# RIKEN-RCCS/GEMMul8

Measured on AMD Instinct MI355X. Metric: emulated DGEMM TFLOPS (N=8192, moduli=14), higher is better.
Workload: dtype int8

## Files before the change

### gemmul8_amd/csrc/oz2_driver.hip

```cpp
#include <hip/hip_runtime.h>
#include <stdint.h>
#include <stdio.h>
#include <stdlib.h>
#include <string.h>

#include <algorithm>

#include <atomic>
#include <mutex>

#include "../../include/gemmul8_c.h"
#include "oz2_gemm_common.hpp"
#include "oz2_kernels.h"
#include "oz2_knobs.hpp"

using namespace oz2;

namespace {

inline char* align256(void* p) {
    uintptr_t x = reinterpret_cast<uintptr_t>(p);
    x = (x + 255) & ~uintptr_t(255);
    return reinterpret_cast<char*>(x);
}
inline int norm_op(int op) {
    if (op >= 111 && op <= 113) return op - 111;
    return op;
}
inline size_t low_size(int) { return 1; }
inline size_t mid_size(int backend, bool cplx) { return (backend == kINT8 ? 1 : 2) * (cplx ? 2 : 1); }

static inline bool moduli_ok(int dtype, unsigned N) { return N >= 2 && N <= (is_f32(dtype) ? 13u : 20u); }

static inline bool f8_concat_ok(size_t k, size_t m, size_t n, size_t kp) { return k <= 32768 && 2 * (m + n) * kp <= ((size_t)384 << 20); }

#define OZ2_HIP(expr)                       \
    do {                                    \
        hipError_t e__ = (expr);            \
        if (e__ != hipSuccess) return (int)e__; \
    } while (0)

struct Timer {
    hipEvent_t ev[4];
    bool made = false, ok = false;
};
Timer* thread_timer() {
    constexpr int kMaxDev = 64;
    static thread_local Timer t[kMaxDev];
    int dev = 0;
    if (hipGetDevice(&dev) != hipSuccess || dev < 0 || dev >= kMaxDev) return nullptr;
    Timer& T = t[dev];
    if (!T.made) {
        T.made = T.ok = true;
        for (auto& e : T.ev)
            if (hipEventCreate(&e) != hipSuccess) T.ok = false;
    }
    return T.ok ? &T : nullptr;
}

}

static bool scalars_on_device(const void* alpha);

namespace oz2 {
static Knobs parse_knobs() {
    Knobs k;
    auto num = [](const char* name, int dflt) {
        const char* s = getenv(name);
        return s && *s ? atoi(s) : dflt;
    };
    if (const char* e = getenv("GEMMUL8_EPI_NT"); e && (e[0] == '0' || e[0] == '1') && !e[1]) k.epi_nt = e[0] - '0';
    if (const int t = num("GEMMUL8_BOUND_TILE", 0); t == 128 || t == 256) k.bound_tile = t;
    if (num("GEMMUL8_CPLX_BOUND_LAUNCHES", 1) == 2) k.cplx_bound_launches = 2;
    if (const int c = num("GEMMUL8_CPLX_CHUNK", 0); c >= 1) k.cplx_chunk = c;
    if (const char* e = getenv("GEMMUL8_CRT_KERNEL")) k.crt_kernel = e[0] == 'd' ? 1 : e[0] == 'r' ? 2 : 0;
    if (const int c = num("GEMMUL8_GEMM_CUS", 0); c >= 8) k.gemm_cus = c & ~7;
    if (const char* e = getenv("GEMMUL8_FP8_FUSED"); e && e[0] == '0') k.fp8_fused = 0;
    if (const char* e = getenv("GEMMUL8_FP8_PLANES")) k.fp8_planes = e[0] == 'e' ? 1 : 0;
    if (const char* e = getenv("GEMMUL8_SCALE_FOLD"); e && e[0] == '0') k.scale_fold = 0;
    if (const char* e = getenv("GEMMUL8_BOUNDS_ONE_READ"); e && (e[0] == '0' || e[0] == '1') && !e[1]) k.bounds_one_read = e[0] - '0';
    if (const char* e = getenv("GEMMUL8_CRT_PANELS"); e && atoi(e) > 1) {
        k.crt_panels = std::min(atoi(e), 256);
        k.crt_panels_ring = e[strlen(e) - 1] == 'r';
    }
    if (const char* e = getenv("GEMMUL8_MAP_COLBLOCK"); e && *e) k.map_colblock = atoi(e) > 0 ? atoi(e) : 0;
    return k;
}
static std::atomic<const Knobs*> g_knobs{nullptr};
static std::mutex g_knobs_mtx;
void reload_knobs() {
    std::lock_guard<std::mutex> lk(g_knobs_mtx);
    g_knobs.store(new Knobs(parse_knobs()), std::memory_order_release);
}
const Knobs& knobs() {
    const Knobs* k = g_knobs.load(std::memory_order_acquire);
    if (!k) {
        std::lock_guard<std::mutex> lk(g_knobs_mtx);
        k = g_knobs.load(std::memory_order_acquire);
        if (!k) g_knobs.store(k = new Knobs(parse_knobs()), std::memory_order_release);
    }
    return *k;
}
}

extern "C" {

void gemmul8_reload_knobs(void) { oz2::reload_knobs(); }

static std::atomic<int> g_nonfinite_mode{0};
int gemmul8_set_nonfinite_mode(int mode) {
    if (mode < 0 || mode > 1) return GEMMUL8_E_ARG;
    return g_nonfinite_mode.exchange(mode);
}

int gemmul8_set_fp8_bound_mode(int mode) {
    if (mode < 0 || mode > 2) return GEMMUL8_E_ARG;
    const int old = get_f8_bound_mode();
    set_f8_bound_mode(mode);
    return old;
}

int gemmul8_abi_version(void) { return GEMMUL8_ABI_VERSION; }
size_t gemmul8_layout_bytes(void) { return sizeof(gemmul8_layout); }

const char* gemmul8_version(void) { return "gemmul8-mi355x 0.5 (gfx950; v_mfma_i32_16x16x64_i8 / v_mfma_scale_f32_16x16x128_f8f6f4, fused epilogues)"; }

size_t gemmul8_work_size(int is_complex, int backend, size_t m, size_t n, size_t k, unsigned N, int enA, int enB, size_t* wA,
                         size_t* wB) {
    const size_t kp = padding256(k), mp = padding256(m);
    const size_t sizeA = kp * mp, sizeB = kp * n, sizeC = mp * n;
    const size_t nm = num_mat(backend, N);
    const size_t parts = is_complex ? 3 : 1;
    const size_t midsz = mid_size(backend, is_complex != 0);
    const size_t nhi = (backend == kINT8 ? 1 : 3) * parts;
    const size_t lwork = size_t(1) << 25;
    size_t tA = 255, tB = 255, tC = 255;
    tA += sizeA * (nm + (enA ? 1 : 0)) * parts + 2 * mp;
    tB += sizeB * (nm + (enB ? 1 : 0)) * parts + 2 * padding256(n);
    tC += midsz * sizeC * (N - 1) + std::max(lwork, midsz * sizeC);
    tC += 4 * sizeC * nhi;
    if (wA) *wA = tA;
    if (wB) *wB = tB;
    return tA + tB + tC;
}

int gemmul8_get_layout(int dtype, int backend, size_t m, size_t n, size_t k, unsigned N, void* work, void* workA, void* workB,
                       int enA, int enB, gemmul8_layout* L) {
    if (!L || !work) return GEMMUL8_E_ARG;
    if (!moduli_ok(dtype, N)) return GEMMUL8_E_NUM_MODULI;
    const bool cplx = is_complex(dtype);
    memset(L, 0, sizeof(*L));
    L->kp = padding256(k);
    L->mp = padding256(m);
    L->num_mat = num_mat(backend, N);
    L->parts = cplx ? 3 : 1;
    L->sizeA = L->kp * L->mp;
    L->sizeB = L->kp * n;
    L->sizeC = L->mp * n;
    const size_t offsetA = L->sizeA * L->num_mat, offsetB = L->sizeB * L->num_mat;
    const size_t size_vecA = L->mp, size_vecB = padding256(n);
    char* w = align256(work);
    char* wa = workA ? align256(workA) : nullptr;
    char* wb = workB ? align256(workB) : nullptr;
    char* A_lo = wa ? wa : w;
    char* sftA = A_lo + L->parts * offsetA + (enA ? L->parts * L->sizeA : 0);
    char* B_lo = wb ? wb : (wa ? w : sftA + 2 * size_vecA);
    char* sftB = B_lo + L->parts * offsetB + (enB ? L->parts * L->sizeB : 0);
    char* C_mid = wb ? (wa ? w : sftA + 2 * size_vecA) : sftB + 2 * size_vecB;
    const size_t midsz = mid_size(backend, cplx);
    char* work_native = C_mid + (N - 1) * L->sizeC * midsz;
    const size_t native_sz = std::max(size_t(1) << 25, midsz * L->sizeC);
    char* C_hi = work_native + native_sz;
    const size_t hi_bytes = 4 * L->sizeC * (backend == kINT8 ? 1 : 3) * L->parts;
    L->A_lo = A_lo;
    L->B_lo = B_lo;
    L->part_strideA = offsetA;
    L->part_strideB = offsetB;
    L->A_bound = enA ? A_lo + L->parts * offsetA : A_lo;
    L->B_bound = enB ? B_lo + L->parts * offsetB : B_lo;
    L->sftA = reinterpret_cast<int16_t*>(sftA);
    L->sftB = reinterpret_cast<int16_t*>(sftB);
    L->C_mid = C_mid;
    const size_t tail = (native_sz - midsz * L->sizeC) & ~size_t(255);
    L->scratch = C_hi - tail;
    L->scratch_bytes = tail + hi_bytes;
    L->lo_format = (backend == kFP8 && !enA && !enB && f6_planes_ok(n)) ? 1 : 0;
    return GEMMUL8_OK;
}

static inline size_t scale_fixed_bytes(size_t mp, size_t np) { return (4 * (mp + np) + 2 * (mp + np) + 255) / 256 * 256; }
static inline size_t scale_scratch_bytes(size_t mp, size_t np) { return scale_fixed_bytes(mp, np) + 8 * (mp + np); }
static int scale_scratch(const gemmul8_layout* L, size_t n, int** rowmax, int** colmax, void** amax, int16_t** s0A = nullptr, int16_t** s0B = nullptr) {
    const size_t np = padding256(n);
    if (L->scratch_bytes < scale_scratch_bytes(L->mp, np)) return GEMMUL8_E_ARG;
    *rowmax = (int*)L->scratch;
    *colmax = *rowmax + L->mp;
    int16_t* s0 = (int16_t*)(*colmax + np);
    if (s0A) *s0A = s0;
    if (s0B) *s0B = s0 + L->mp;
    *amax = (char*)L->scratch + scale_fixed_bytes(L->mp, np);
    return GEMMUL8_OK;
}

static int bound_gemm_i8(hipStream_t stream, bool cplx, const gemmul8_layout* L, size_t m, size_t ncols, const int8_t* Ab, const int8_t* Bb, int* rowmax, int* colmax) {
    if (!cplx) {
        const int8_t* As[1] = {Ab};
        const int8_t* Bs[1] = {Bb};
        OZ2_HIP(launch_gemm_i8_max(stream, 1, As, Bs, L->kp, m, ncols, rowmax, colmax));
    } else {
        const int8_t* As[3] = {Ab, Ab + L->sizeA, Ab + 2 * L->sizeA};
        const int8_t* Bs[3] = {Bb + L->sizeB, Bb, Bb + 2 * L->sizeB};
        const bool two_launches = knobs().cplx_bound_launches == 2;
        if (two_launches) {
            OZ2_HIP(launch_gemm_i8_max(stream, 2, As, Bs, L->kp, m, ncols, rowmax, colmax));
            OZ2_HIP(launch_gemm_i8_max(stream, 3, As, Bs, L->kp, m, ncols, rowmax, colmax));
        } else {
            OZ2_HIP(launch_gemm_i8_max(stream, 3, As, Bs, L->kp, m, ncols, rowmax, colmax, 2));
        }
    }
    return GEMMUL8_OK;
}

struct SymSide {
    bool onB;
    int form;
    bool herm;
    bool conj = false;
};
constexpr size_t kOneReadMinRows = 8192;
static int scale_bounds_nf(void* stream_, int dtype, int backend, int op_A, int op_B, size_t m, size_t n, size_t k, const void* A, size_t lda,
                           const void* B, size_t ldb, unsigned N, size_t col_begin, size_t col_end, const gemmul8_layout* L, int skipA, int skipB,
                           bool nf, const SymSide* sym = nullptr) {
    hipStream_t stream = (hipStream_t)stream_;
// ... 893 lines not shown
```

### gemmul8_amd/csrc/oz2_knobs.hpp

```cpp
#pragma once

namespace oz2 {

struct Knobs {
    int epi_nt = -1;
    int bound_tile = 0;
    int cplx_bound_launches = 1;
    int cplx_chunk = 0;
    int crt_kernel = 0;
    int fp8_planes = 0;
    int fp8_fused = 1;
    int gemm_cus = 0;
    int crt_panels = 0;
    int crt_panels_ring = 0;
    int scale_fold = 1;
    int bounds_one_read = -1;
    int map_colblock = -1;
};
const Knobs& knobs();
void reload_knobs();

}
```

### gemmul8_amd/csrc/oz2_scale.hip

```cpp
#include <hip/hip_runtime.h>
#include <limits.h>
#include <stdint.h>

#include <algorithm>
#include <type_traits>

#include "oz2_kernels.h"

namespace oz2 {

ModTable make_mod_table(int backend) {
    ModTable T;
    for (int t = 0; t < 20; ++t) {
        const int p = backend == kINT8 ? GEMMUL8_MODULI_INT8[t] : GEMMUL8_MODULI_FP8[t];
        T.mc[t].p = p;
        T.mc[t].invp = 1.0f / (float)p;
        unsigned c[16];
        long long pw = 1;
        for (int i = 0; i < 16; ++i) {
            c[i] = i < 15 ? (unsigned)(pw % p) : 0u;
            pw = (pw % p) * 256;
        }
        for (int i = 0; i < 4; ++i) {
            unsigned lo = 0, hi = 0;
// ... 780 lines not shown
                    for (int e = 0; e < RPL; ++e) {
                        const T q = (lrow + e < a.rows) ? x[kg * a.ld + e] : (T)0;
                        __builtin_memcpy((char*)&v + e * sizeof(T), &q, sizeof(T));
                    }
                }
            }
            b[it] = v;
        }
    };
    auto to_lds = [&](const V4 (&b)[NL]) {
#pragma unroll
        for (int it = 0; it < NL; ++it) {
            const int kk = ky + KY * it;
#pragma unroll
            for (int e = 0; e < RPL; ++e) __builtin_memcpy(&tile[RPL * rp + e][kk], (const char*)&b[it] + e * sizeof(T), sizeof(T));
        }
    };
    auto consume = [&]<bool FAST>(unsigned t) {
#pragma unroll
        for (int p = 0; p < NP; ++p) {
            const int rl = p * RPP + rg;
            T v[4];
            T lm = 0;
#pragma unroll
            for (int e = 0; e < 4; ++e) {
                v[e] = tile[rl][c * 4 + e];
                const T ax = sizeof(T) == 8 ? (T)fabs((double)v[e]) : (T)fabsf((float)v[e]);
                lm = ax > lm ? ax : lm;
                if constexpr (sizeof(T) == 8) {
                    const unsigned hw = (unsigned)__double2hiint((double)ax);
                    mnk[p] = (v[e] != (T)0 && hw < mnk[p]) ? hw : mnk[p];
                }
            }
            int key = lm == (T)0 ? kNone : lm == (T)INFINITY ? INT_MAX : ilogb0(lm);
#pragma unroll
            for (int off = CH / 2; off > 0; off >>= 1) key = max(key, __shfl_xor(key, off));
            const int prev = ex[p];
            ex[p] = max(prev, key);
            if (c == 0) step[rl][t] = (unsigned char)(prev == kNone ? 0 : min(min(ex[p], 4096) - min(prev, 4096), 255));
            if (FAST || r0 + rl < a.rows) emit4<T, MODE_BOUND>(a, r0 + rl, (size_t)t * TK + c * 4, v, ex[p] == kNone ? 5 : 5 - min(ex[p], 4096));
        }
    };
    unsigned tdone = 0;
    if (r0 + TR <= a.rows && ((reinterpret_cast<uintptr_t>(X + r0) | (a.ld * sizeof(T))) & 15u) == 0) {
        auto fetch = [&](unsigned t, V4 (&b)[NL]) {
#pragma unroll
            for (int it = 0; it < NL; ++it) b[it] = __builtin_nontemporal_load((const V4*)(x + ((size_t)t * TK + ky + KY * it) * a.ld));
        };
        V4 buf[D][NL];
#pragma unroll
        for (int j = 0; j < D; ++j) {
#pragma unroll
            for (int it = 0; it < NL; ++it) buf[j][it] = V4{0u, 0u, 0u, 0u};
            if ((unsigned)j < nfull) fetch((unsigned)j, buf[j]);
        }
        for (unsigned t0 = 0; t0 < nfull; t0 += D) {
#pragma unroll
            for (int j = 0; j < D; ++j) {
                const unsigned t = t0 + j;
                if (t < nfull) {
                    to_lds(buf[j]);
                    if (t + D < nfull) fetch(t + D, buf[j]);
                    __syncthreads();
                    consume.template operator()<true>(t);
                    __syncthreads();
                }
            }
        }
        tdone = nfull;
    }
    for (unsigned t = tdone; t < nkt; ++t) {
        V4 b[NL];
        fetch_guarded(t, b);
        to_lds(b);
        __syncthreads();
        consume.template operator()<false>(t);
        __syncthreads();
    }
#pragma unroll
    for (int p = 0; p < NP; ++p) {
        const int rl = p * RPP + rg;
        const size_t row = r0 + rl;
        if (row >= a.rows) continue;
        const int s0 = ex[p] == kNone ? 5 : ex[p] == INT_MAX ? 5 - ilogb0((T)INFINITY) : 5 - ex[p];
        if (c == 0) {
            ((int16_t*)((char*)a.sft0 + OZ2_ZW))[row] = (int16_t)s0;
            if (a.sft0_keep) ((int16_t*)((char*)a.sft0_keep + OZ2_ZW))[row] = (int16_t)s0;
        }
        bool hazard = ex[p] == INT_MAX;
        if constexpr (sizeof(T) == 8) {
            unsigned mk = mnk[p];
#pragma unroll
            for (int off = CH / 2; off > 0; off >>= 1) mk = min(mk, (unsigned)__shfl_xor((int)mk, off));
            const int emin = (mk >> 20) == 0 ? -1074 : (int)(mk >> 20) - 1023;
            hazard = hazard || (ex[p] != kNone && mk != 0xFFFFFFFFu && s0 + emin < -1022);
        }
        if (hazard) {
            for (unsigned t = 0; t < nkt; ++t) {
                const size_t k0 = (size_t)t * TK + c * 4;
                T v[4];
#pragma unroll
                for (int e = 0; e < 4; ++e) v[e] = (k0 + e < a.k) ? X[(k0 + e) * a.ld + row] : (T)0;
                emit4<T, MODE_BOUND>(a, row, k0, v, s0);
            }
            continue;
        }
        unsigned d = 0;
        for (int t = (int)nkt - 1; t >= 1; --t) {
            d = min(d + step[rl][t], 64u);
            if (d == 0) continue;
            unsigned* q = (unsigned*)(a.lo + OZ2_ZW + row * a.kp + (size_t)(t - 1) * TK + c * 4);
            const unsigned w = *q;
            *q = d >= 8 ? (((w + 0x7F7F7F7Fu) >> 7) & 0x01010101u) : (((w + ((1u << d) - 1u) * 0x01010101u) >> d) & ((0xFFu >> d) * 0x01010101u));
        }
    }
}

template <typename T> __global__ void __launch_bounds__(256) extract_pair_kernel(const StageArgs a, const StageArgs b, const unsigned nA, const int kmA, const int kmB) {
    if (a.zero_words) {
        unsigned* zp = (unsigned*)((char*)a.zero_p + OZ2_ZW);
        for (unsigned i = blockIdx.x * 256u + threadIdx.x; i < a.zero_words; i += gridDim.x * 256u) zp[i] = 0u;
    }
    if (blockIdx.x < nA) {
        if (kmA) stage_kmajor_body<T, MODE_BOUND>(a, blockIdx.x);
        else stage_strided_body<T, MODE_BOUND>(a, blockIdx.x);
    } else {
        if (kmB) stage_kmajor_body<T, MODE_BOUND>(b, blockIdx.x - nA);
        else stage_strided_body<T, MODE_BOUND>(b, blockIdx.x - nA);
    }
}
enum { FORM_STRIDED = 0, FORM_KMAJOR = 1, FORM_PANEL = 2 };
template <typename T> __device__ __forceinline__ void extract_body(const StageArgs& a, const unsigned bid, const int form) {
    if (form == FORM_KMAJOR) return stage_kmajor_body<T, MODE_BOUND>(a, bid);
    if (form == FORM_PANEL) return stage_panel_body<T>(a, bid);
    stage_strided_body<T, MODE_BOUND>(a, bid);
}
template <typename T> __global__ void __launch_bounds__(256) extract_panel_pair_kernel(const StageArgs a, const StageArgs b, const unsigned nA, const int fA, const int fB) {
    if (a.zero_words) {
        unsigned* zp = (unsigned*)((char*)a.zero_p + OZ2_ZW);
        for (unsigned i = blockIdx.x * 256u + threadIdx.x; i < a.zero_words; i += gridDim.x * 256u) zp[i] = 0u;
    }
    if (blockIdx.x < nA) extract_body<T>(a, blockIdx.x, fA);
    else extract_body<T>(b, blockIdx.x - nA, fB);
}
template <typename T> __global__ void __launch_bounds__(256) quantise_pair_kernel(const StageArgs a, const StageArgs b, const unsigned nA, const int kmA, const int kmB) {
    if (blockIdx.x < nA) {
        if (kmA) stage_kmajor_body<T, MODE_MOD>(a, blockIdx.x);
        else stage_strided_body<T, MODE_MOD>(a, blockIdx.x);
    } else {
        if (kmB) stage_kmajor_body<T, MODE_MOD>(b, blockIdx.x - nA);
        else stage_strided_body<T, MODE_MOD>(b, blockIdx.x - nA);
    }
}
template <typename T> __global__ void __launch_bounds__(256) quantise_twin_kernel(const StageArgs a, const int km) {
    static_assert(ET<T>::cplx, "complex operands");
    if (km) stage_kmajor_body<T, MODE_MOD, true>(a, blockIdx.x);
    else stage_strided_body<T, MODE_MOD, true>(a, blockIdx.x);
}
template <typename T> __global__ void __launch_bounds__(256) extract_seg2_kernel(const StageArgs a, const int km) {
    if (a.zero_words) {
        unsigned* zp = (unsigned*)((char*)a.zero_p + OZ2_ZW);
        for (unsigned i = blockIdx.x * 256u + threadIdx.x; i < a.zero_words; i += gridDim.x * 256u) zp[i] = 0u;
    }
    if (km) stage_kmajor_seg2_body<T, MODE_BOUND>(a, blockIdx.x);
    else stage_strided_body<T, MODE_BOUND, false, true>(a, blockIdx.x);
}
template <typename T> __global__ void __launch_bounds__(256) quantise_seg2_kernel(const StageArgs a, const int km) {
    if (km) stage_kmajor_seg2_body<T, MODE_MOD>(a, blockIdx.x);
    else stage_strided_body<T, MODE_MOD, false, true>(a, blockIdx.x);
}
static_assert(2 * sizeof(StageArgs) + 16 <= 4096, "two argument blocks must fit the 4 KiB kernel-argument segment");

typedef float v16f __attribute__((ext_vector_type(16)));
typedef unsigned v6u __attribute__((ext_vector_type(6)));
template <typename T> __device__ __forceinline__ void stage_f6_body(const StageArgs& a, const unsigned bid, const bool kmajor, char* tile ) {
    static_assert(!ET<T>::cplx, "real operands");
    constexpr int EPL = 16 / (int)sizeof(T);
    constexpr int CH = 128 / (int)sizeof(T);
    const unsigned lane = threadIdx.x & 63u, q = threadIdx.x >> 6;
    const unsigned nks = (unsigned)(a.kp / 128), nrb = (unsigned)((a.rows + 63) / 64);
    unsigned rb, kt;
    if (kmajor) rb = bid / nks, kt = bid - rb * nks;
    else kt = bid / nrb, rb = bid - kt * nrb;
    const size_t r0 = (size_t)rb * 64, row = r0 + lane, k0 = (size_t)kt * 128 + (size_t)q * 32;
    const T* X = (const T*)((const char*)a.X + OZ2_ZX);
    typedef unsigned V4 __attribute__((ext_vector_type(4)));
    T v[32];
    if (kmajor) {
        const unsigned pc = lane & 7u, pr = lane >> 3;
#pragma unroll
        for (int c = 0; c < 32 / CH; ++c) {
            V4 buf[8];
#pragma unroll
            for (int j = 0; j < 8; ++j) {
                const size_t r = r0 + pr + 8 * j, kk = k0 + (size_t)c * CH + (size_t)pc * EPL;
                const T* src = X + r * a.ld + kk;
                V4 t = {0u, 0u, 0u, 0u};
                if (r < a.rows) {
                    if (kk + EPL <= a.k && (reinterpret_cast<uintptr_t>(src) & 15u) == 0) {
                        t = __builtin_nontemporal_load((const V4*)src);
                    } else {
                        T e[EPL];
#pragma unroll
                        for (int u = 0; u < EPL; ++u) e[u] = kk + u < a.k ? src[u] : ET<T>::zero();
                        __builtin_memcpy(&t, e, 16);
                    }
                }
                buf[j] = t;
            }
            if (c > 0) __builtin_amdgcn_wave_barrier();
#pragma unroll
            for (int j = 0; j < 8; ++j) *(V4*)(tile + (pr + 8 * j) * 144 + pc * 16) = buf[j];
            __builtin_amdgcn_wave_barrier();
#pragma unroll
            for (int i = 0; i < 8; ++i) {
                const V4 t = *(const V4*)(tile + lane * 144 + i * 16);
                __builtin_memcpy(&v[c * CH + i * EPL], &t, 16);
            }
        }
    } else {
        const T* src = X + row;
#pragma unroll
        for (int kk = 0; kk < 32; ++kk) {
            const size_t kg = k0 + kk;
            v[kk] = (row < a.rows && kg < a.k) ? __builtin_nontemporal_load(src + kg * a.ld) : ET<T>::zero();
        }
    }
    if (row >= a.rows) return;
    int s = OZ2_ROW_SHIFT(a, row, k0 == 0);
    if (a.nf && s == kNonfiniteShift) {
#pragma unroll
        for (int e = 0; e < 32; ++e) v[e] = ET<T>::zero();
        s = 0;
    }
    using XS = typename std::conditional<sizeof(T) == 4, float, double>::type;
    XS xs[32];
    bool big = false;
#pragma unroll
    for (int e = 0; e < 32; ++e) {
        if constexpr (sizeof(T) == 4) xs[e] = truncf(ldexpf(v[e], s));
        else xs[e] = trunc(ldexp((double)v[e], s));
        big |= fabs((double)xs[e]) >= 0x1.0p53;
    }
    const unsigned tb = (unsigned)(row >> 8), r = (unsigned)row & 255u;
    const unsigned rp = tb == a.f6_last ? a.f6_rp_last : 256u;
    int8_t* const panel = a.lo + OZ2_ZW + (size_t)tb * 256u * (a.kp / 4 * 3) + (size_t)kt * rp * 96u;
    int8_t* const ox = panel + (size_t)(q * rp + r) * 16u;
    int8_t* const oy = panel + 64u * (size_t)rp + (size_t)((q >> 1) * 2u * rp + 2u * r + (q & 1u)) * 8u;
    auto put = [&](int plane, const float (&w)[32]) {
        v16f ev, od;
#pragma unroll
        for (int i = 0; i < 16; ++i) ev[i] = w[2 * i], od[i] = w[2 * i + 1];
        const v6u c = __builtin_amdgcn_cvt_scalef32_2xpk16_fp6_f32(ev, od, 8.0f);
        typedef unsigned V2 __attribute__((ext_vector_type(2)));
        *(V4*)(ox + (size_t)plane * a.plane_stride) = V4{c[0], c[1], c[2], c[3]};
        *(V2*)(oy + (size_t)plane * a.plane_stride) = V2{c[4], c[5]};
    };
    auto run = [&]<bool BIG>() {
        for (int t = a.t_begin; t < a.t_end; t += 2) {
            const double P = a.pairP[(t - a.t_begin) >> 1], invP = a.pairInvP[(t - a.t_begin) >> 1];
            float Rf[32];
#pragma unroll
            for (int g8 = 0; g8 < 4; ++g8) {
#pragma unroll
                for (int e = 8 * g8; e < 8 * g8 + 8; ++e) {
                    const double x = (double)xs[e];
                    double R = fma(-rint(x * invP), P, x);
                    if constexpr (BIG) R = fma(-rint(R * invP), P, R);
                    Rf[e] = (float)R;
                }
                __builtin_amdgcn_sched_barrier(0);
            }
#pragma unroll 1
            for (int u = 0; u < 2; ++u) {
                const int tt = t + u;
                if (tt >= a.t_end) break;
                const ModConst mc = a.mt.mc[tt];
                const float pf = (float)mc.p;
                const bool even = !(mc.p & 1);
                const bool sqm = tt < 6;
                float lo[32], hi[32];
                if (even) {
                    asm volatile("" ::: "memory");
#pragma unroll
                    for (int e = 0; e < 32; ++e) {
                        const float qq = fmaf(Rf[e], mc.invp, 12582912.0f) - 12582912.0f;
                        const float rr = fmaf(-qq, pf, Rf[e]);
                        lo[e] = rr == -0.5f * pf ? 0.5f * pf : rr;
                    }
                } else {
#pragma unroll
                    for (int g8 = 0; g8 < 4; ++g8) {
#pragma unroll
                        for (int e = 8 * g8; e < 8 * g8 + 8; ++e) {
                            const float qq = fmaf(Rf[e], mc.invp, 12582912.0f) - 12582912.0f;
                            lo[e] = fmaf(-qq, pf, Rf[e]);
                        }
                        __builtin_amdgcn_sched_barrier(0);
                    }
                }
                if (sqm) {
                    const float sq = (float)a.sqrtp[tt], inv = 1.0f / sq;
#pragma unroll
                    for (int g8 = 0; g8 < 4; ++g8) {
#pragma unroll
                        for (int e = 8 * g8; e < 8 * g8 + 8; ++e) {
// ... 187 lines not shown
    };
    const AmaxOperand a = mk(A), b = mk(B);
    const size_t nA = (size_t)a.row_groups * a.parts, nB = (size_t)b.row_groups * b.parts;
    if (nA + nB == 0) return hipSuccess;
    if (nA + nB > 0x7FFFFFFFull) return hipErrorInvalidConfiguration;
    hipLaunchKernelGGL(amax_pair_kernel<T>, dim3((unsigned)(nA + nB), 1, g_batch.batch), dim3(256), 0, stream, a, b, (unsigned)nA, k, g_batch.ws);
    return hipGetLastError();
}
static hipError_t launch_amax_sym_pair(hipStream_t stream, int dtype, size_t k, const ExtractOperand& A, const ExtractOperand& B);
static hipError_t launch_extract_sym_pair(hipStream_t stream, int dtype, int backend, size_t k, size_t kp, const ExtractOperand& A, const ExtractOperand& B,
                                          void* zero_p, size_t zero_bytes);
static hipError_t launch_fast_shift_sym_pair(hipStream_t stream, int dtype, int backend, unsigned N, size_t k, const QuantOperand& A, const QuantOperand& B);
static hipError_t launch_quantise_sym_pair(hipStream_t stream, int dtype, int backend, int t_begin, int t_end, size_t k, size_t kp, const QuantOperand& A,
                                           const QuantOperand& B);

hipError_t launch_amax_pair(hipStream_t stream, int dtype, size_t k, const ExtractOperand& A, const ExtractOperand& B) {
    if (A.sym || B.sym) return launch_amax_sym_pair(stream, dtype, k, A, B);
    switch (dtype) {
    case kF32: return launch_amax_pair_t<float>(stream, k, A, B);
    case kF64: return launch_amax_pair_t<double>(stream, k, A, B);
    case kC32: return launch_amax_pair_t<float2>(stream, k, A, B);
    case kC64: return launch_amax_pair_t<double2>(stream, k, A, B);
    }
    return hipErrorInvalidValue;
}
template <typename T> static size_t extract_blocks(int form, const StageArgs& a) {
    if (form == FORM_PANEL) return (a.rows + StageTile<T>::TR - 1) / StageTile<T>::TR;
    return stage_blocks<T, MODE_BOUND>(form == FORM_KMAJOR, a);
}
template <typename T> static hipError_t launch_extract_pair_t(hipStream_t stream, int kmA, StageArgs a, int kmB, const StageArgs& b, void* zero_p, size_t zero_bytes) {
    const size_t nA = extract_blocks<T>(kmA, a), nB = extract_blocks<T>(kmB, b);
    if (nA + nB == 0) return zero_bytes ? launch_zero(stream, zero_p, zero_bytes) : hipSuccess;
    if (nA + nB > 0x7FFFFFFFull) return hipErrorInvalidConfiguration;
    if (zero_p && zero_bytes) a.zero_p = (unsigned*)zero_p, a.zero_words = (unsigned)(zero_bytes / 4);
    if constexpr (!ET<T>::cplx) {
        if (kmA == FORM_PANEL || kmB == FORM_PANEL) {
            hipLaunchKernelGGL(extract_panel_pair_kernel<T>, dim3((unsigned)(nA + nB), 1, g_batch.batch), dim3(256), 0, stream, a, b, (unsigned)nA, kmA, kmB);
            return hipGetLastError();
        }
    }
    hipLaunchKernelGGL(extract_pair_kernel<T>, dim3((unsigned)(nA + nB), 1, g_batch.batch), dim3(256), 0, stream, a, b, (unsigned)nA, kmA, kmB);
    return hipGetLastError();
}
bool extract_one_read_ok(int dtype, int backend, size_t kp) {
    return (dtype == kF32 || dtype == kF64) && backend == kINT8 && g_batch.batch == 1 && kp / StageTile<double>::TK <= (size_t)kPanelMaxTiles;
}
hipError_t launch_extract_pair(hipStream_t stream, int dtype, int backend, size_t k, size_t kp, const ExtractOperand& A, const ExtractOperand& B, void* zero_p,
                               size_t zero_bytes) {
    if (A.sym || B.sym) return launch_extract_sym_pair(stream, dtype, backend, k, kp, A, B, zero_p, zero_bytes);
    const StageArgs a = extract_args(backend, k, kp, A), b = extract_args(backend, k, kp, B);
    auto form = [&](const ExtractOperand& o) { return o.kmajor ? FORM_KMAJOR : o.one_read ? FORM_PANEL : FORM_STRIDED; };
    if ((A.one_read || B.one_read) && !extract_one_read_ok(dtype, backend, kp)) return hipErrorInvalidValue;
    const int fA = form(A), fB = form(B);
    switch (dtype) {
    case kF32: return launch_extract_pair_t<float>(stream, fA, a, fB, b, zero_p, zero_bytes);
    case kF64: return launch_extract_pair_t<double>(stream, fA, a, fB, b, zero_p, zero_bytes);
    case kC32: return launch_extract_pair_t<float2>(stream, fA, a, fB, b, zero_p, zero_bytes);
    case kC64: return launch_extract_pair_t<double2>(stream, fA, a, fB, b, zero_p, zero_bytes);
    }
    return hipErrorInvalidValue;
}

static StageArgs quantise_args(int backend, int t_begin, int t_end, size_t k, size_t kp, const QuantOperand& o) {
    StageArgs a{};
    a.bx = o.xstride;
    a.bw = g_batch.ws;
    a.X = o.X;
    a.ld = o.ld;
    a.rows = o.rows;
    a.k = k;
    a.kp = kp;
    a.lo = o.lo;
    a.plane_stride = o.plane_stride;
    a.part_stride = o.part_stride;
    a.sft = o.sft;
    if (o.fin_max) {
        a.fin_sft0 = o.fin_sft0;
        a.fin_max = o.fin_max;
        a.fin_out = o.sft;
        a.fin_log2P = o.fin_log2P;
        a.fin_float_max = backend == kFP8 ? 1 : 0;
    }
    a.backend = backend;
    a.conj = o.conj;
    a.nf = o.nf ? 1 : 0;
    a.t_begin = t_begin;
    a.t_end = t_end;
    a.mt = make_mod_table(backend);
    for (int t = t_begin, j = 0; t < t_end && j < 10; t += 2, ++j) {
        const double P = (double)a.mt.mc[t].p * (t + 1 < t_end ? (double)a.mt.mc[t + 1].p : 1.0);
        a.pairP[j] = P;
        a.pairInvP[j] = 1.0 / P;
    }
    for (int t = 0; t < 6; ++t) a.sqrtp[t] = GEMMUL8_SQRT_MODULI_FP8[t];
    if (backend == kFP8 && o.f6_rows > 0) {
        a.f6 = 1;
        a.f6_last = (unsigned)((o.f6_rows - 1) / 256);
        a.f6_rp_last = (unsigned)((o.f6_rows - 256 * (size_t)a.f6_last + 15) / 16 * 16);
    }
    return a;
}

static hipError_t launch_quantise_twin(hipStream_t stream, int dtype, int t_begin, int t_end, size_t k, size_t kp, const QuantOperand& A) {
    StageArgs a = quantise_args(kINT8, t_begin, t_end, k, kp, A);
    a.lo2 = A.lo2, a.plane_stride2 = A.plane_stride2, a.part_stride2 = A.part_stride2;
    const size_t nA = dtype == kC32 ? stage_blocks<float2, MODE_MOD>(A.kmajor, a) : stage_blocks<double2, MODE_MOD>(A.kmajor, a);
    if (nA > 0x7FFFFFFFull) return hipErrorInvalidConfiguration;
    const dim3 grid((unsigned)nA, 1, g_batch.batch);
    if (dtype == kC32) hipLaunchKernelGGL(quantise_twin_kernel<float2>, grid, dim3(256), 0, stream, a, (int)A.kmajor);
    else hipLaunchKernelGGL(quantise_twin_kernel<double2>, grid, dim3(256), 0, stream, a, (int)A.kmajor);
    return hipGetLastError();
}

template <typename T, int MODE> static size_t seg2_blocks(bool kmajor, const StageArgs& a) {
    if (kmajor) return a.rows * ((MODE == MODE_MOD && sizeof(T) <= 8) ? 2 * ((a.kp + 1023) / 1024) : 1);
    return 2 * (a.kp / StageTile<T>::TK) * ((a.rows + StageTile<T>::TR - 1) / StageTile<T>::TR);
}
static void seg2_args(StageArgs& a, size_t kp, const Seg2Planes& S) {
    a.X2 = S.X2, a.ld2 = S.ld2, a.pitch = 2 * kp;
    a.lo2 = S.lo2, a.plane_stride2 = S.plane_stride2, a.part_stride2 = S.part_stride2;
}
template <typename T, int MODE> static hipError_t launch_seg2_t(hipStream_t stream, bool kmajor, const StageArgs& a) {
    const size_t nb = seg2_blocks<T, MODE>(kmajor, a);
    if (nb == 0 || nb > 0x7FFFFFFFull) return hipErrorInvalidConfiguration;
    if constexpr (MODE == MODE_BOUND) hipLaunchKernelGGL(extract_seg2_kernel<T>, dim3((unsigned)nb), dim3(256), 0, stream, a, (int)kmajor);
    else hipLaunchKernelGGL(quantise_seg2_kernel<T>, dim3((unsigned)nb), dim3(256), 0, stream, a, (int)kmajor);
    return hipGetLastError();
}
template <int MODE> static hipError_t launch_seg2(hipStream_t stream, int dtype, bool kmajor, const StageArgs& a) {
    if (g_batch.batch != 1 || a.rows == 0 || a.kp % 256 != 0 || !a.X2 || !a.lo2) return hipErrorInvalidValue;
    switch (dtype) {
    case kF32: return launch_seg2_t<float, MODE>(stream, kmajor, a);
    case kF64: return launch_seg2_t<double, MODE>(stream, kmajor, a);
    case kC32: return launch_seg2_t<float2, MODE>(stream, kmajor, a);
    case kC64: return launch_seg2_t<double2, MODE>(stream, kmajor, a);
    }
    return hipErrorInvalidValue;
}
hipError_t launch_extract_seg2(hipStream_t stream, int dtype, size_t k, size_t kp, const ExtractOperand& A, const Seg2Planes& S, void* zero_p, size_t zero_bytes) {
    if (A.one_read || A.conj) return hipErrorInvalidValue;
    StageArgs a = extract_args(kINT8, k, kp, A);
    seg2_args(a, kp, S);
    if (zero_p && zero_bytes) a.zero_p = (unsigned*)zero_p, a.zero_words = (unsigned)(zero_bytes / 4);
    return launch_seg2<MODE_BOUND>(stream, dtype, A.kmajor, a);
}
hipError_t launch_quantise_seg2(hipStream_t stream, int dtype, int t_begin, int t_end, size_t k, size_t kp, const QuantOperand& A, const Seg2Planes& S) {
    if (t_end <= t_begin) return hipSuccess;
    if (A.conj || A.f6_rows || A.nf || A.lo2) return hipErrorInvalidValue;
    StageArgs a = quantise_args(kINT8, t_begin, t_end, k, kp, A);
    seg2_args(a, kp, S);
    return launch_seg2<MODE_MOD>(stream, dtype, A.kmajor, a);
}

hipError_t launch_quantise_pair(hipStream_t stream, int dtype, int backend, int t_begin, int t_end, size_t k, size_t kp, const QuantOperand& A,
                                const QuantOperand& B) {
    if ((A.rows == 0 && B.rows == 0) || t_end <= t_begin) return hipSuccess;
    if (A.sym || B.sym) return launch_quantise_sym_pair(stream, dtype, backend, t_begin, t_end, k, kp, A, B);
    if (A.lo2 || B.lo2) {
        if (B.rows || B.lo2 || A.rows == 0 || !is_complex(dtype) || backend != kINT8 || A.f6_rows || A.nf) return hipErrorInvalidValue;
        return launch_quantise_twin(stream, dtype, t_begin, t_end, k, kp, A);
    }
    const StageArgs a = quantise_args(backend, t_begin, t_end, k, kp, A), b = quantise_args(backend, t_begin, t_end, k, kp, B);
    switch (dtype) {
    case kF32: return launch_quantise_stage<float>(stream, A.kmajor, a, B.kmajor, b);
    case kF64: return launch_quantise_stage<double>(stream, A.kmajor, a, B.kmajor, b);
    case kC32: return launch_quantise_stage<float2>(stream, A.kmajor, a, B.kmajor, b);
    case kC64: return launch_quantise_stage<double2>(stream, A.kmajor, a, B.kmajor, b);
    }
    return hipErrorInvalidValue;
}

__global__ void shift_finalize_kernel(size_t rowsA, const int* maxA, int16_t* sftA, unsigned blocksA, size_t rowsB, const int* maxB,
                                      int16_t* sftB, float log2P, int float_max, size_t bw, int nf) {
    {
        const size_t o = blockIdx.z * bw;
        maxA = (const int*)((const char*)maxA + o), maxB = (const int*)((const char*)maxB + o);
        sftA = (int16_t*)((char*)sftA + o), sftB = (int16_t*)((char*)sftB + o);
    }
    const bool isB = blockIdx.x >= blocksA;
    const size_t r = (size_t)(isB ? blockIdx.x - blocksA : blockIdx.x) * blockDim.x + threadIdx.x;
    if (r >= (isB ? rowsB : rowsA)) return;
    const int amax = (isB ? maxB : maxA)[r];
    int f = 0;
    if (amax > 0) {
        const float l = __log2f(float_max ? __int_as_float(amax) : __int2float_rn(amax));
        f = __float2int_rd(__fmaf_rd(-0x1.000006p-1f, l, log2P));
    }
    int16_t* sft = isB ? sftB : sftA;
    if (nf && sft[r] == kNonfiniteSft) return;
    sft[r] = (int16_t)(-((int)sft[r] + f));
}
hipError_t launch_shift_finalize(hipStream_t stream, int backend, unsigned N, size_t rowsA, const int* maxA, int16_t* sftA, size_t rowsB,
                                 const int* maxB, int16_t* sftB, bool nf) {
    const unsigned bA = (unsigned)((rowsA + 255) / 256), bB = (unsigned)((rowsB + 255) / 256);
    if (bA + bB == 0) return hipSuccess;
    const float log2P = backend == kINT8 ? GEMMUL8_LOG2P_INT8[N - 2] : GEMMUL8_LOG2P_FP8[N - 2];
    hipLaunchKernelGGL(shift_finalize_kernel, dim3(bA + bB, 1, g_batch.batch), dim3(256), 0, stream, rowsA, maxA, sftA, bA, rowsB, maxB, sftB, log2P,
                       backend == kFP8 ? 1 : 0, g_batch.ws, nf ? 1 : 0);
    return hipGetLastError();
}

template <typename U> __device__ __forceinline__ U add_ru(U a, U b);
template <> __device__ __forceinline__ float add_ru<float>(float a, float b) { return __fadd_ru(a, b); }
template <> __device__ __forceinline__ double add_ru<double>(double a, double b) { return __dadd_ru(a, b); }
template <typename U> __device__ __forceinline__ U sqr_add_ru(U x, U s);
template <> __device__ __forceinline__ float sqr_add_ru<float>(float x, float s) { return __fmaf_ru(x, x, s); }
template <> __device__ __forceinline__ double sqr_add_ru<double>(double x, double s) { return __fma_ru(x, x, s); }

template <typename U> __device__ __forceinline__ U tree32_sum_ru(U v) {
#pragma unroll
    for (int off = 16; off > 0; off >>= 1) v = add_ru<U>(v, __shfl_down(v, off, 32));
    return v;
}
template <typename U> __device__ __forceinline__ U tree32_max(U v) {
#pragma unroll
    for (int off = 16; off > 0; off >>= 1) {
        const U o = __shfl_down(v, off, 32);
        v = o > v ? o : v;
    }
    return v;
}

__device__ __forceinline__ int fast_sft(double amax, double vecnrm, float log2P) {
    const int exponent = ilogb0(vecnrm);
    const float vecnrmf = __double2float_ru(scalbn(vecnrm, -exponent));
    const float log2vsum = __fadd_ru(__log2f(vecnrmf), (float)exponent);
    const float log2vnrm = __fmul_ru(0x1.000006p-1f, log2vsum);
    const float exp1 = __fsub_rd(__fsub_rd(log2P, 1.5f), fmaxf(1.0f, log2vnrm));
    return __float2int_rd(exp1) - ilogb0((float)amax);
}
__device__ __forceinline__ int fast_sft(float amax, float vecnrm, float log2P) {
    const float log2vsum = __log2f(vecnrm);
    const float log2vnrm = __fmul_ru(0x1.000006p-1f, log2vsum);
    const float exp1 = __fsub_rd(__fsub_rd(log2P, 1.5f), fmaxf(1.0f, log2vnrm));
    return __float2int_rd(exp1) - ilogb0(amax);
}

template <typename T, bool SEG2 = false>
__device__ __forceinline__ void fast_shift_kmajor_body(const T* X, size_t ld, size_t k, int16_t* sft, float log2P, const unsigned bid, [[maybe_unused]] const T* X2 = nullptr,
                                                       [[maybe_unused]] size_t ld2 = 0) {
    using E = ET<T>;
    using U = typename E::U;
    __shared__ U samax[32], ssum[32];
    U amax = 0, sum = 0;
    auto segment = [&](const T* x) {
        size_t i = threadIdx.x;
        for (; i + 3 * 256 < k; i += 4 * 256) {
            T v[4];
#pragma unroll
            for (int u = 0; u < 4; ++u) v[u] = x[i + 256 * u];
#pragma unroll
            for (int u = 0; u < 4; ++u) {
                const U ar = (U)fabs(E::re(v[u]));
                amax = ar > amax ? ar : amax;
                sum = sqr_add_ru<U>(ar, sum);
                if constexpr (E::cplx) {
                    const U ai = (U)fabs(E::im(v[u]));
                    amax = ai > amax ? ai : amax;
                    sum = sqr_add_ru<U>(ai, sum);
                }
            }
        }
        for (; i < k; i += 256) {
            const T v = x[i];
            const U ar = (U)fabs(E::re(v));
            amax = ar > amax ? ar : amax;
            sum = sqr_add_ru<U>(ar, sum);
            if constexpr (E::cplx) {
                const U ai = (U)fabs(E::im(v));
                amax = ai > amax ? ai : amax;
                sum = sqr_add_ru<U>(ai, sum);
            }
        }
    };
    segment(X + (size_t)bid * ld);
    if constexpr (SEG2) segment(X2 + (size_t)bid * ld2);
    amax = tree32_max(amax);
    sum = tree32_sum_ru(sum);
    if ((threadIdx.x & 31) == 0) {
        samax[threadIdx.x >> 5] = amax;
        ssum[threadIdx.x >> 5] = sum;
    }
    __syncthreads();
    if (threadIdx.x < 32) {
        amax = threadIdx.x < 8 ? samax[threadIdx.x] : (U)0;
        sum = threadIdx.x < 8 ? ssum[threadIdx.x] : (U)0;
        amax = tree32_max(amax);
        sum = tree32_sum_ru(sum);
        if (threadIdx.x == 0) sft[bid] = (int16_t)(-fast_sft(amax, sum, log2P));
    }
}

template <typename T, bool SEG2 = false>
__device__ __forceinline__ void fast_shift_strided_body(const T* X, size_t ld, size_t rows, size_t k, int16_t* sft, float log2P, const unsigned bid,
                                                        [[maybe_unused]] const T* X2 = nullptr, [[maybe_unused]] size_t ld2 = 0) {
    using E = ET<T>;
    using U = typename E::U;
    constexpr int RPL = 16 / (int)sizeof(T), RPB = 8 * RPL;
    __shared__ U samax[32][RPB + 1], ssum[32][RPB + 1];
    const int tx = threadIdx.x & 7, ty = threadIdx.x >> 3;
    const size_t row0 = (size_t)bid * RPB + (size_t)tx * RPL;
    U amax[RPL], sum[RPL];
#pragma unroll
    for (int j = 0; j < RPL; ++j) amax[j] = 0, sum[j] = 0;
    auto take = [&](const T& v, int j) {
        const U ar = (U)fabs(E::re(v));
        amax[j] = ar > amax[j] ? ar : amax[j];
        sum[j] = sqr_add_ru<U>(ar, sum[j]);
        if constexpr (E::cplx) {
            const U ai = (U)fabs(E::im(v));
            amax[j] = ai > amax[j] ? ai : amax[j];
            sum[j] = sqr_add_ru<U>(ai, sum[j]);
        }
    };
    auto segment = [&](const T* Xs, const size_t lds) {
// ... 619 lines not shown
```

Measured before the change: 159.5.

## Add streaming quantise kernel with run-based prefetch and nontemporal loads for large real GEMMs

Adds a new quantise path for real f32/f64 INT8 operands in which each block processes a run of several consecutive k-chunks or row tiles. While the current chunk is being emitted, the next chunk is prefetched into registers with nontemporal vector loads. It is selected automatically when k and the row counts are at least 8192, or it can be forced through an environment knob. The aim is to hide global-load latency and cut cache pollution during quantisation. In exchange the launch uses fewer blocks, which can reduce parallelism, and the prefetch buffers add register pressure.

New measurement: 160.4, median of 6. Within noise of the previous version (+0.6%).

```diff
diff --git a/gemmul8_amd/csrc/oz2_driver.hip b/gemmul8_amd/csrc/oz2_driver.hip
--- a/gemmul8_amd/csrc/oz2_driver.hip
+++ b/gemmul8_amd/csrc/oz2_driver.hip
@@ -79,6 +79,7 @@
     if (const char* e = getenv("GEMMUL8_FP8_PLANES")) k.fp8_planes = e[0] == 'e' ? 1 : 0;
     if (const char* e = getenv("GEMMUL8_SCALE_FOLD"); e && e[0] == '0') k.scale_fold = 0;
     if (const char* e = getenv("GEMMUL8_BOUNDS_ONE_READ"); e && (e[0] == '0' || e[0] == '1') && !e[1]) k.bounds_one_read = e[0] - '0';
+    if (const char* e = getenv("GEMMUL8_QUANT_STREAM"); e && (e[0] == '0' || e[0] == '1') && !e[1]) k.quant_stream = e[0] - '0';
     if (const char* e = getenv("GEMMUL8_CRT_PANELS"); e && atoi(e) > 1) {
         k.crt_panels = std::min(atoi(e), 256);
         k.crt_panels_ring = e[strlen(e) - 1] == 'r';
diff --git a/gemmul8_amd/csrc/oz2_knobs.hpp b/gemmul8_amd/csrc/oz2_knobs.hpp
--- a/gemmul8_amd/csrc/oz2_knobs.hpp
+++ b/gemmul8_amd/csrc/oz2_knobs.hpp
@@ -15,6 +15,7 @@
     int crt_panels_ring = 0;
     int scale_fold = 1;
     int bounds_one_read = -1;
+    int quant_stream = -1;
     int map_colblock = -1;
 };
 const Knobs& knobs();
diff --git a/gemmul8_amd/csrc/oz2_scale.hip b/gemmul8_amd/csrc/oz2_scale.hip
--- a/gemmul8_amd/csrc/oz2_scale.hip
+++ b/gemmul8_amd/csrc/oz2_scale.hip
@@ -956,6 +956,134 @@
         else stage_strided_body<T, MODE_MOD>(b, blockIdx.x - nA);
     }
 }
+#ifndef OZ2_STREAM_RUN
+#define OZ2_STREAM_RUN 4
+#endif
+constexpr int kStreamRun = OZ2_STREAM_RUN;
+typedef unsigned StreamV4 __attribute__((ext_vector_type(4)));
+template <int NV> __device__ __forceinline__ void stream_issue(StreamV4 (&r)[NV], const void* p, size_t step) {
+#pragma unroll
+    for (int q = 0; q < NV; ++q) r[q] = __builtin_nontemporal_load((const StreamV4*)((const char*)p + q * step));
+}
+template <typename T> __device__ __forceinline__ void stream_kmajor_body(const StageArgs& a, const unsigned bid) {
+    constexpr int S = kStreamRun;
+    constexpr int NQ = (int)(4 * sizeof(T) / 16);
+    const unsigned nch = (unsigned)(a.kp / 1024 + (a.kp % 1024 != 0));
+    const unsigned nrun = (nch + S - 1) / S;
+    const unsigned rowu = bid / nrun;
+    const size_t row = rowu;
+    const unsigned c0 = (bid - rowu * nrun) * S;
+    const T* x = (const T*)a.X + row * a.ld;
+    const int s = OZ2_ROW_SHIFT(a, row, c0 == 0 && threadIdx.x == 0);
+    const unsigned nin = (unsigned)(a.k / 1024);
+    const int nit = (int)(nch - c0 < (unsigned)S ? nch - c0 : (unsigned)S);
+    int nfull = 0;
+    if ((reinterpret_cast<uintptr_t>(x) & 15u) == 0 && nin > c0) nfull = (int)(nin - c0 < (unsigned)S ? nin - c0 : (unsigned)S);
+    const size_t kt = (size_t)c0 * 1024 + (size_t)threadIdx.x * 4;
+    StreamV4 ring[NQ] = {};
+    if (nfull > 0) stream_issue<NQ>(ring, x + kt, 16);
+#pragma unroll 1
+    for (int i = 0; i < nit; ++i) {
+        const size_t k0 = kt + (size_t)i * 1024;
+        T v[4];
+        if (i < nfull) {
+            __builtin_memcpy(v, ring, sizeof(ring));
+        } else {
+            if (k0 >= a.kp) break;
+            load4<T>(x, k0, a.k, v);
+#pragma unroll
+            for (int e = 0; e < 4; ++e) asm volatile("" : "+v"(v[e]));
+        }
+        if (i + 1 < nfull) stream_issue<NQ>(ring, x + k0 + 1024, 16);
+        emit4<T, MODE_MOD>(a, row, k0, v, s);
+    }
+}
+template <typename T> __device__ __forceinline__ void stream_strided_body(const StageArgs& a, const unsigned bid) {
+    using E = ET<T>;
+    constexpr int S = kStreamRun;
+    constexpr int TR = StageTile<T>::TR, TK = StageTile<T>::TK;
+    constexpr int PITCH = TK + 16 / (int)sizeof(T);
+    constexpr int CH = TK / 4, RPP = 256 / CH, NP = TR / RPP;
+    constexpr int RPL = 16 / (int)sizeof(T), RP = TR / RPL, KY = 256 / RP, NL = TK / KY;
+    static_assert(S * TR <= 256, "one thread per row of the run");
+    __shared__ __attribute__((aligned(16))) T tile[TR][PITCH];
+    __shared__ int shl[S * TR];
+    const unsigned nrt = (unsigned)((a.rows + TR - 1) / TR);
+    const unsigned nrun = (nrt + S - 1) / S;
+    const unsigned kt = bid / nrun, rt0 = (bid - kt * nrun) * S;
+    const size_t kb = (size_t)kt * TK;
+    const int nit = (int)(nrt - rt0 < (unsigned)S ? nrt - rt0 : (unsigned)S);
+    const unsigned nfr = (unsigned)(a.rows / TR);
+    int nfull = 0;
+    if (kb + TK <= a.k && ((reinterpret_cast<uintptr_t>(a.X) | (a.ld * sizeof(T))) & 15u) == 0 && nfr > rt0)
+        nfull = (int)(nfr - rt0 < (unsigned)S ? nfr - rt0 : (unsigned)S);
+    const int rp = threadIdx.x % RP, ky = threadIdx.x / RP;
+    const int c = threadIdx.x % CH;
+    const T* const xk = (const T*)a.X + (kb + ky) * a.ld + RPL * rp;
+    const size_t step = (size_t)KY * a.ld * sizeof(T);
+    StreamV4 cur[NL] = {};
+    if (nfull > 0) stream_issue<NL>(cur, xk + (size_t)rt0 * TR, step);
+    if (threadIdx.x < S * TR) {
+        const size_t row = (size_t)rt0 * TR + threadIdx.x;
+        if (row < a.rows) shl[threadIdx.x] = OZ2_ROW_SHIFT(a, row, kt == 0);
+    }
+#pragma unroll 1
+    for (int i = 0; i < nit; ++i) {
+        const size_t r0 = (size_t)(rt0 + i) * TR;
+        if (i >= nfull) {
+            const size_t row = r0 + RPL * rp;
+            const T* x = (const T*)a.X + row;
+            const bool pair_ok = row + RPL - 1 < a.rows && ((reinterpret_cast<uintptr_t>(x) | (a.ld * sizeof(T))) & 15u) == 0;
+#pragma unroll
+            for (int it = 0; it < NL; ++it) {
+                const size_t kg = kb + ky + KY * it;
+                StreamV4 v = {0u, 0u, 0u, 0u};
+                if (kg < a.k) {
+                    if (pair_ok) {
+                        v = __builtin_nontemporal_load((const StreamV4*)(x + kg * a.ld));
+                    } else {
+#pragma unroll
+                        for (int e = 0; e < RPL; ++e) {
+                            const T t = (row + e < a.rows) ? x[kg * a.ld + e] : E::zero();
+                            __builtin_memcpy((char*)&v + e * sizeof(T), &t, sizeof(T));
+                        }
+                    }
+                }
+                cur[it] = v;
+            }
+        }
+        if (i > 0) __syncthreads();
+#pragma unroll
+        for (int it = 0; it < NL; ++it) {
+            const int kk = ky + KY * it;
+#pragma unroll
+            for (int e = 0; e < RPL; ++e) __builtin_memcpy(&tile[RPL * rp + e][kk], (const char*)&cur[it] + e * sizeof(T), sizeof(T));
+        }
+        __syncthreads();
+        if (i + 1 < nfull) stream_issue<NL>(cur, xk + (r0 + TR), step);
+#pragma unroll 1
+        for (int pass = 0; pass < NP; ++pass) {
+            const int rl = pass * RPP + threadIdx.x / CH;
+            const size_t row = r0 + rl;
+            if (row >= a.rows) continue;
+            const int s = shl[i * TR + rl];
+            T v[4];
+#pragma unroll
+            for (int e = 0; e < 4; ++e) v[e] = tile[rl][c * 4 + e];
+            emit4<T, MODE_MOD>(a, row, kb + c * 4, v, s);
+        }
+    }
+}
+template <typename T> __global__ void __launch_bounds__(256) quantise_stream_pair_kernel(const StageArgs a, const StageArgs b, const unsigned nA, const int kmA, const int kmB) {
+    static_assert(!ET<T>::cplx, "real operands");
+    if (blockIdx.x < nA) {
+        if (kmA) stream_kmajor_body<T>(a, blockIdx.x);
+        else stream_strided_body<T>(a, blockIdx.x);
+    } else {
+        if (kmB) stream_kmajor_body<T>(b, blockIdx.x - nA);
+        else stream_strided_body<T>(b, blockIdx.x - nA);
+    }
+}
 template <typename T> __global__ void __launch_bounds__(256) quantise_twin_kernel(const StageArgs a, const int km) {
     static_assert(ET<T>::cplx, "complex operands");
     if (km) stage_kmajor_body<T, MODE_MOD, true>(a, blockIdx.x);
@@ -1449,6 +1577,26 @@
     return launch_seg2<MODE_MOD>(stream, dtype, A.kmajor, a);
 }
 
+template <typename T> static size_t stream_blocks(bool kmajor, const StageArgs& a) {
+    if (a.rows == 0) return 0;
+    if (kmajor) return a.rows * (((a.kp + 1023) / 1024 + kStreamRun - 1) / kStreamRun);
+    return (a.kp / StageTile<T>::TK) * (((a.rows + StageTile<T>::TR - 1) / StageTile<T>::TR + kStreamRun - 1) / kStreamRun);
+}
+template <typename T> static hipError_t launch_quantise_stream(hipStream_t stream, bool kmA, const StageArgs& a, bool kmB, const StageArgs& b) {
+    const size_t nA = stream_blocks<T>(kmA, a), nB = stream_blocks<T>(kmB, b);
+    if (nA + nB == 0) return hipSuccess;
+    if (nA + nB > 0x7FFFFFFFull) return hipErrorInvalidConfiguration;
+    hipLaunchKernelGGL(quantise_stream_pair_kernel<T>, dim3((unsigned)(nA + nB)), dim3(256), 0, stream, a, b, (unsigned)nA, (int)kmA, (int)kmB);
+    return hipGetLastError();
+}
+constexpr size_t kStreamMinRows = 8192, kStreamMinK = 8192;
+static bool quantise_stream_taken(int dtype, int backend, size_t k, const QuantOperand& A, const QuantOperand& B) {
+    if (!(dtype == kF32 || dtype == kF64) || backend != kINT8 || g_batch.batch != 1 || A.f6_rows || B.f6_rows) return false;
+    const int force = knobs().quant_stream;
+    if (force >= 0) return force == 1;
+    return k >= kStreamMinK && (A.rows == 0 || A.rows >= kStreamMinRows) && (B.rows == 0 || B.rows >= kStreamMinRows);
+}
+
 hipError_t launch_quantise_pair(hipStream_t stream, int dtype, int backend, int t_begin, int t_end, size_t k, size_t kp, const QuantOperand& A,
                                 const QuantOperand& B) {
     if ((A.rows == 0 && B.rows == 0) || t_end <= t_begin) return hipSuccess;
@@ -1458,6 +1606,8 @@
         return launch_quantise_twin(stream, dtype, t_begin, t_end, k, kp, A);
     }
     const StageArgs a = quantise_args(backend, t_begin, t_end, k, kp, A), b = quantise_args(backend, t_begin, t_end, k, kp, B);
+    if (quantise_stream_taken(dtype, backend, k, A, B))
+        return dtype == kF32 ? launch_quantise_stream<float>(stream, A.kmajor, a, B.kmajor, b) : launch_quantise_stream<double>(stream, A.kmajor, a, B.kmajor, b);
     switch (dtype) {
     case kF32: return launch_quantise_stage<float>(stream, A.kmajor, a, B.kmajor, b);
     case kF64: return launch_quantise_stage<double>(stream, A.kmajor, a, B.kmajor, b);
```
